# rust-bio/rust-bio

Measured on AMD Instinct MI355X. Metric: GCUPS (SW) + FM-index queries/sec, higher is better.
Workload: dtype int16; 1 GPU; 1000000 x 150 bp synthetic read pairs per GPU, Aligner::local affine-gap (-5,-1,+1,-1), score+coords+traceback ops (BASELINE configs[1]); pairs_per_gpu=1000000, read_len=150, parallelism=shard1

## Files before the change

### rust-bio_amd/csrc/bg_common.h

```cpp
#ifndef BG_COMMON_H
#define BG_COMMON_H
#include <functional>
#include <hip/hip_runtime.h>

#include <cstdint>
#include <cstdlib>
#include <cstdio>
#include <cstring>
#include <string>
#include <vector>

#include "biogpu.h"

extern thread_local std::string bg_tls_error;

#define BG_HIP(call)                                                                     \
    do {                                                                                 \
        hipError_t e__ = (call);                                                         \
        if (e__ != hipSuccess) {                                                         \
            bg_tls_error = std::string(#call) + ": " + hipGetErrorString(e__);           \
            return e__ == hipErrorOutOfMemory ? BG_ERR_OOM : BG_ERR_HIP;                 \
        }                                                                                \
    } while (0)

struct bg_band_scratch;
void bg_band_scratch_free(bg_band_scratch*);
struct bg_seed_scratch;
void bg_seed_scratch_free(bg_seed_scratch*);
struct bg_host_pipe;
void bg_host_pipe_free(bg_host_pipe*);
struct bg_fm_pipe;
void bg_fm_pipe_free(bg_fm_pipe*);
struct bg_myers_scratch;
void bg_myers_scratch_free(bg_myers_scratch*);

struct bg_ctx {
    int device = 0;
    hipStream_t stream = nullptr;
    void* tb = nullptr;
    size_t tb_bytes = 0;
    void* aux = nullptr;
    size_t aux_bytes = 0;
    void* bnd = nullptr;
    size_t bnd_bytes = 0;
    void* io[6] = {};
    size_t io_cap[6] = {};
    void* h_ops = nullptr;
    size_t h_ops_cap = 0;
    void* unpk[2] = {};
    size_t unpk_cap[2] = {};
    void* table = nullptr;
    size_t table_bytes = 0;
    void* sw_table = nullptr;
    size_t sw_table_bytes = 0;
    uint64_t table_hash = 0;
    int table_alpha = 0;
    int32_t* table_matrix = nullptr;
    bg_band_scratch* band = nullptr;
    bg_host_pipe* pipe = nullptr;
    bg_seed_scratch* seed = nullptr;
    bg_fm_pipe* fm_pipe = nullptr;
    bg_myers_scratch* myers = nullptr;
    int64_t myers_chunk_jobs = 0;
    int64_t myers_lds_bytes = 0;
    uint64_t fm_wide_from = 0xFFFFFFFFull;
    uint32_t fm_wide_sb_shift = 17;
    bool fm_host_bytes = false;
    int64_t host_chunk_pairs = 0;
    int64_t chunk_pairs = 0;
    int64_t seed_chunk_reads = 0;
    bool force_wide = false;
    bool no_pk16 = false;
    bool no_local_fast = false;
    bool no_pk16_frame = false;
    bool no_couples = false;
    int band_chain_global = -1;
    bool fq_no_fused = false;
    int sam_lanes = 0;
    int64_t sa_chunk_symbols = 0;
    bool band_chain_rows = true;
    bool band_join_global = false;
    int band_fill_v1 = 0;
    bool band_interior_off = false;
    bool band_packed_off = false;
    int64_t band_packed_thresh = 0;
    int64_t band_budget_gb = 0;
    bool band_on_host = false;
    hipEvent_t scratch_done = nullptr;
    hipStream_t scratch_stream = nullptr;
    bool scratch_used = false;
    bool timing = false;
    hipEvent_t ev[2] = {nullptr, nullptr};
    bg_timing_t last = {};
    uint32_t fill_mask = 0;
    bool fill_framed = false;
};

int bg_reserve(void** p, size_t* cur, size_t need);
int bg_scan_u32(const uint32_t* d_len, uint64_t n, uint64_t* d_off, uint64_t* d_sums, hipStream_t st);
int bg_align_batch_dev_hint(bg_ctx* ctx, const bg_scoring_t* sc, int mode, uint64_t n_pairs, const uint8_t* d_x,
                            const uint64_t* d_x_off, const uint8_t* d_y, const uint64_t* d_y_off, uint32_t max_xlen,
                            uint32_t max_ylen, bg_alignment_t* d_out, uint8_t* d_ops, uint64_t ops_stride, void* stream,
                            int len_hint);

size_t bg_compact_ops_scratch(uint64_t n);
int bg_range_to_host(const uint8_t* d_src, uint8_t* h_dst, const uint64_t* d_slot , hipStream_t st);
int bg_compact_ops_dev(bg_alignment_t* d_rec, uint64_t n, const uint8_t* d_ops, uint8_t* d_compact, bool global_offsets, uint64_t* d_cell,
                       uint64_t* d_batch_total, void* d_scratch, bool long_ops, hipStream_t st);

struct bg_scratch_guard {
    bg_ctx* ctx;
    hipStream_t st;
    bg_scratch_guard(bg_ctx* c, hipStream_t s) : ctx(c), st(s) {
        if (ctx->scratch_used && ctx->scratch_stream != st) hipStreamWaitEvent(st, ctx->scratch_done, 0);
    }
    ~bg_scratch_guard() {
        if (hipEventRecord(ctx->scratch_done, st) == hipSuccess) {
            ctx->scratch_stream = st;
            ctx->scratch_used = true;
        }
    }
};
inline hipError_t bg_copy_pieces(void* dst, const void* src, size_t bytes, hipMemcpyKind kind, hipStream_t st) {
    static const size_t piece = [] {
        const char* e = getenv("BG_COPY_PIECE");
        const long long v = e ? atoll(e) : 0;
        return v > 0 ? (size_t)v : (size_t)(8u << 20);
// ... 29 lines not shown
```

### rust-bio_amd/csrc/core.hip

```cpp
#include <sched.h>

#include <algorithm>
#include <condition_variable>
#include <deque>
#include <mutex>
#include <thread>

#include <cstdlib>

#include "bg_common.h"

thread_local std::string bg_tls_error;

int bg_reserve(void** p, size_t* cur, size_t need) {
    if (need <= *cur) return BG_OK;
    if (*p) {
        hipFree(*p);
        *p = nullptr;
        *cur = 0;
    }
    need = (need + 255) & ~(size_t)255;
    BG_HIP(hipMalloc(p, need));
    *cur = need;
    return BG_OK;
// ... 205 lines not shown
        ctx->band_chain_rows = value != 0;
        return BG_OK;
    }
    if (!strcmp(key, "band_chain_global")) {
        ctx->band_chain_global = (int)value;
        return BG_OK;
    }
    if (!strcmp(key, "band_fill_v1")) {
        ctx->band_fill_v1 = value > 0 ? 1 : value < 0 ? -1 : 0;
        return BG_OK;
    }
    if (!strcmp(key, "band_interior_off")) {
        ctx->band_interior_off = value != 0;
        return BG_OK;
    }
    if (!strcmp(key, "band_packed_off")) {
        ctx->band_packed_off = value != 0;
        return BG_OK;
    }
    if (!strcmp(key, "band_packed_thresh")) {
        if (value < 0 || value > 0xffff) return BG_ERR_INVALID_ARG;
        ctx->band_packed_thresh = value;
        return BG_OK;
    }
    if (!strcmp(key, "band_budget_gb")) {
        if (value < 0 || value > 256) return BG_ERR_INVALID_ARG;
        ctx->band_budget_gb = value;
        return BG_OK;
    }
    if (!strcmp(key, "band_on_host")) {
        ctx->band_on_host = value != 0;
        return BG_OK;
    }
    if (!strcmp(key, "fm_host_bytes")) {
        ctx->fm_host_bytes = value != 0;
        return BG_OK;
    }
    if (!strcmp(key, "host_chunk_pairs")) {
        ctx->host_chunk_pairs = value;
        return BG_OK;
    }
    if (!strcmp(key, "no_couples")) {
        ctx->no_couples = value != 0;
        return BG_OK;
    }
    if (!strcmp(key, "no_local_fast")) {
        ctx->no_local_fast = value != 0;
        return BG_OK;
    }
    if (!strcmp(key, "no_pk16_frame")) {
        ctx->no_pk16_frame = value != 0;
        return BG_OK;
    }
    if (!strcmp(key, "no_pk16")) {
        ctx->no_pk16 = value != 0;
        return BG_OK;
    }
    if (!strcmp(key, "force_wide")) {
        ctx->force_wide = value != 0;
        return BG_OK;
    }
    return BG_ERR_INVALID_ARG;
}

extern "C" int bg_enable_timing(bg_ctx* ctx, int on) {
    if (!ctx) return BG_ERR_INVALID_ARG;
    ctx->timing = on != 0;
    ctx->last = {};
    return BG_OK;
}

extern "C" int bg_last_fill_kernels(bg_ctx* ctx, uint32_t* mask) {
    if (!ctx || !mask) return BG_ERR_INVALID_ARG;
    *mask = ctx->fill_mask;
    return BG_OK;
}

extern "C" int bg_last_fill_framed(bg_ctx* ctx, int* framed) {
    if (!ctx || !framed) return BG_ERR_INVALID_ARG;
    *framed = ctx->fill_framed ? 1 : 0;
    return BG_OK;
}

extern "C" int bg_get_timing(bg_ctx* ctx, bg_timing_t* out) {
    if (!ctx || !out) return BG_ERR_INVALID_ARG;
    *out = ctx->last;
    ctx->last = {};
    return BG_OK;
}

namespace {
__global__ __launch_bounds__(256) void ops_counts_kernel(const bg_alignment_t* __restrict__ rec, uint64_t n, uint32_t* __restrict__ cnt) {
    const uint64_t p = (uint64_t)blockIdx.x * blockDim.x + threadIdx.x;
    if (p < n) cnt[p] = rec[p].status == BG_OK ? rec[p].n_ops : 0u;
}
template <int LANES>
__global__ __launch_bounds__(256) void ops_compact_kernel(bg_alignment_t* __restrict__ rec, uint64_t n, const uint8_t* __restrict__ ops,
                                                          const uint64_t* __restrict__ off, const uint64_t* __restrict__ cell,
                                                          uint8_t* __restrict__ compact, int global_offsets) {
    const uint64_t p = ((uint64_t)blockIdx.x * blockDim.x + threadIdx.x) / LANES;
    const uint32_t l = threadIdx.x % LANES;
    if (p >= n) return;
    const uint32_t k = rec[p].status == BG_OK ? rec[p].n_ops : 0u;
    const uint64_t base = *cell;
    const uint8_t* src = ops + rec[p].ops_off;
    uint8_t* dst = compact + (global_offsets ? base : 0ull) + off[p];
// ... 50 lines not shown
```

### rust-bio_amd/csrc/sw_api.hip

```cpp
#include <algorithm>
#include <chrono>
#include <map>
#include <type_traits>

#include <atomic>
#include <condition_variable>
#include <mutex>
#include <thread>

#include "sw_kernels.h"

namespace bgsw {
void launch_traceback(const SwArgs& a, int nw, hipStream_t st);

static sw_fill_fn sw_fill_get(SwFill f, bool narrow, int lp, int r, int which = 0) {
    static sw_fill_fn (*const get[])(bool, int, int, int) = {
#define BG_X(F) sw_fill_get_##F,
        BG_SW_FILLS(BG_X)
#undef BG_X
    };
    return get[f](narrow, lp, r, which);
}
static int instantiated_r(SwFill f, bool narrow, int lp, int r0, uint32_t m = 0) {
    for (int r = r0; r <= 12; r++)
        if ((!m || m % r == 0) && sw_fill_get(f, narrow, lp, r)) return r;
    return 0;
}

struct Config {
    int lp, r;
};
static Config pick_config(uint32_t m_cap) {
    if (m_cap <= 192) return {16, std::max(2, 2 * (int)((m_cap + 31) / 32))};
    if (m_cap <= 384) return {32, std::max(8, 2 * (int)((m_cap + 63) / 64))};
    return {64, 8};
}

static int64_t score_magnitude(const SwScoring& c, const int32_t* matrix) {
    int64_t mag = std::max<int64_t>(std::abs((int64_t)c.go), std::abs((int64_t)c.ge));
    for (int32_t v : {c.xp, c.xs, c.yp, c.ys})
        if (v != BG_MIN_SCORE) mag = std::max<int64_t>(mag, std::abs((int64_t)v));
    if (matrix) {
        for (size_t t = 0; t < 65536; t++) mag = std::max<int64_t>(mag, std::abs((int64_t)matrix[t]));
    } else {
        mag = std::max<int64_t>(mag, std::max(std::abs((int64_t)c.match), std::abs((int64_t)c.mismatch)));
    }
    return mag;
}

struct FillPlan {
    int lp = 0, r = 0;
    sw_fill_fn fill = nullptr, fill_rest = nullptr, fill_second = nullptr;
    uint32_t tb_fmt = TBF_K1;
    uint32_t fill_bit = 0;
    bool k1p = false, framed = false;
};
static FillPlan plan_fill(const bg_ctx& ctx, const SwScoring& c, int sm, int64_t mag, uint32_t max_xlen, uint32_t max_ylen) {
    const Config cfg = pick_config(max_xlen);
    const bool local = c.xp == 0 && c.xs == 0 && c.yp == 0 && c.ys == 0;
    const bool lf = local && c.go < 0 && c.mismatch < 0 && c.match >= 0 && !ctx.no_local_fast;
    FillPlan p;
    p.lp = cfg.lp;
    if (!ctx.no_pk16 && sm == SCORE_PARAMS && cfg.lp <= 32 && max_xlen >= 1 && mag * ((int64_t)std::max(max_xlen, max_ylen) + 2) <= 2040) {
        const int32_t M = BG_MIN_SCORE;
        SwFill f = lf      ? FILL_K1P_LF
                   : local ? FILL_K1P_LOCAL
// ... 181 lines not shown
using namespace bgsw;

int bg_compact_matrix(const int32_t* matrix, std::vector<uint8_t>& code_map, std::vector<int32_t>& table) {
    return compact_matrix(matrix, code_map, table);
}

static int check_scoring(const bg_scoring_t* sc) {
    if (sc->gap_open > 0 || sc->gap_extend > 0 || sc->xclip_prefix > 0 || sc->xclip_suffix > 0 ||
        sc->yclip_prefix > 0 || sc->yclip_suffix > 0)
        return BG_ERR_POSITIVE_PENALTY;
    return BG_OK;
}

static void reset_fill_report(bg_ctx* ctx) {
    if (!ctx) return;
    ctx->fill_mask = 0;
    ctx->fill_framed = false;
}

static int align_batch_dev_impl(bg_ctx* ctx, const bg_scoring_t* sc, int mode, uint64_t n_pairs,
                                const uint8_t* d_x, const uint64_t* d_x_off, const uint8_t* d_y,
                                const uint64_t* d_y_off, uint32_t max_xlen, uint32_t max_ylen,
                                bg_alignment_t* d_out, uint8_t* d_ops, uint64_t ops_stride,
                                void* stream, int len_hint, const uint8_t* packed_codes = nullptr) {
    if (!ctx || !sc || mode < BG_MODE_CUSTOM || mode > BG_MODE_LOCAL) return BG_ERR_INVALID_ARG;
    int rc = check_scoring(sc);
    if (rc) return rc;
    if (n_pairs == 0) return BG_OK;
    if (!d_x_off || !d_y_off || !d_out) return BG_ERR_INVALID_ARG;
    if (d_ops && ops_stride < (uint64_t)max_xlen + max_ylen + 4) return BG_ERR_OPS_CAP;
    if (max_xlen > (1u << 24) || max_ylen > (1u << 24)) return BG_ERR_TOO_LARGE;
    hipStream_t st = (hipStream_t)stream;
    BG_HIP(hipSetDevice(ctx->device));
    bg_scratch_guard guard(ctx, st);

    SwArgs a = {};
    a.x = d_x;
    a.x_off = d_x_off;
    a.y = d_y;
    a.y_off = d_y_off;
    a.sc = {sc->gap_open,     sc->gap_extend,   sc->xclip_prefix, sc->xclip_suffix,
            sc->yclip_prefix, sc->yclip_suffix, sc->match_score,  sc->mismatch_score};
    if (mode == BG_MODE_GLOBAL) a.sc.xp = a.sc.xs = a.sc.yp = a.sc.ys = BG_MIN_SCORE;
    if (mode == BG_MODE_SEMIGLOBAL) {
        a.sc.xp = a.sc.xs = BG_MIN_SCORE;
        a.sc.yp = a.sc.ys = 0;
    }
    if (mode == BG_MODE_LOCAL) a.sc.xp = a.sc.xs = a.sc.yp = a.sc.ys = 0;
    a.mode = mode;
    a.filter_clips = (mode == BG_MODE_SEMIGLOBAL || mode == BG_MODE_LOCAL);
    a.out = d_out;
    a.ops = d_ops;
    a.ops_stride = ops_stride;

    int sm = SCORE_PARAMS;
    if (sc->matrix) {
        uint64_t h = 0xcbf29ce484222325ull;
        {
            const uint64_t* w = (const uint64_t*)sc->matrix;
            uint64_t h2 = 0x9e3779b97f4a7c15ull;
            for (size_t t = 0; t < 32768; t += 2) {
                h = (h ^ w[t]) * 0x100000001b3ull;
                h2 = (h2 + w[t + 1]) * 0xff51afd7ed558ccdull;
                h2 ^= h2 >> 32;
            }
            h ^= h2;
            if (h == 0) h = 1;
        }
        if (ctx->table_hash != h || !ctx->table_matrix || memcmp(ctx->table_matrix, sc->matrix, 65536 * sizeof(int32_t)) != 0) {
            std::vector<uint8_t> code_map;
            std::vector<int32_t> table;
            const int A = compact_matrix(sc->matrix, code_map, table);
            const size_t bytes = 256 + table.size() * 4;
            ctx->table_hash = 0;
            if (!ctx->table_matrix && !(ctx->table_matrix = (int32_t*)malloc(65536 * sizeof(int32_t)))) return BG_ERR_OOM;
            if ((rc = bg_reserve(&ctx->sw_table, &ctx->sw_table_bytes, bytes))) return rc;
            BG_HIP(hipMemcpyAsync((uint8_t*)ctx->sw_table + 256, table.data(), table.size() * 4,
                                  hipMemcpyHostToDevice, st));
            BG_HIP(hipMemcpyAsync(ctx->sw_table, code_map.data(), 256, hipMemcpyHostToDevice, st));
            BG_HIP(hipStreamSynchronize(st));
            memcpy(ctx->table_matrix, sc->matrix, 65536 * sizeof(int32_t));
            ctx->table_hash = h;
            ctx->table_alpha = A;
        }
        const int A = ctx->table_alpha;
        sm = A <= kMaxLdsAlphabet ? SCORE_LDS : SCORE_GLOBAL;
        a.code_map = (const uint8_t*)ctx->sw_table;
        a.table = (const int32_t*)((uint8_t*)ctx->sw_table + 256);
        a.alpha = A;
    }

    const FillPlan plan = plan_fill(*ctx, a.sc, sm, score_magnitude(a.sc, sc->matrix), max_xlen, max_ylen);
    if (!plan.fill) return BG_ERR_UNSUPPORTED;
    ctx->fill_mask |= plan.fill_bit;
    if (plan.framed) ctx->fill_framed = true;
    if (packed_codes) {
        if (plan.k1p) {
            a.packed = 1;
        } else {
            uint64_t tot[2] = {0, 0};
            BG_HIP(hipMemcpyAsync(&tot[0], d_x_off + n_pairs, 8, hipMemcpyDeviceToHost, st));
            BG_HIP(hipMemcpyAsync(&tot[1], d_y_off + n_pairs, 8, hipMemcpyDeviceToHost, st));
            BG_HIP(hipStreamSynchronize(st));
            for (int k = 0; k < 2; k++)
                if ((rc = bg_reserve(&ctx->unpk[k], &ctx->unpk_cap[k], std::max<uint64_t>(tot[k], 16)))) return rc;
            if ((rc = bg_unpack2_dev(ctx, (const uint32_t*)d_x, tot[0], packed_codes, (uint8_t*)ctx->unpk[0], st))) return rc;
            if ((rc = bg_unpack2_dev(ctx, (const uint32_t*)d_y, tot[1], packed_codes, (uint8_t*)ctx->unpk[1], st))) return rc;
            a.x = (const uint8_t*)ctx->unpk[0];
            a.y = (const uint8_t*)ctx->unpk[1];
        }
    }
    const int nw = tb_words(plan.r);
    const uint32_t pw = 64 / plan.lp;
    SwGeom& g = a.g;
    g.lp = plan.lp;
    g.r = plan.r;
    g.tb_fmt = plan.tb_fmt;
    g.r_inv = (uint32_t)(((1ull << 32) + plan.r - 1) / plan.r);
    g.lp_shift = plan.lp == 16 ? 4 : plan.lp == 32 ? 5 : 6;
    g.m_cap = max_xlen;
    g.n_cap = max_ylen;
    g.nsteps = max_ylen ? max_ylen + plan.lp - 1 : 0;
    g.nstrips = std::max<uint32_t>(1, (max_xlen + plan.lp * plan.r - 1) / (plan.lp * plan.r));
    g.aux_stride = SwGeom::stride_for(max_xlen, max_ylen);

    const size_t tb_per_job = (size_t)tb_job_words(g.nstrips, g.nsteps, nw) * 4;
    const size_t aux_per_pair = (size_t)g.aux_stride * 4;
    const size_t bnd_per_pair = g.nstrips > 1 ? (size_t)(g.n_cap + 1) * 16 : 0;
    const size_t per_pair = tb_per_job / pw + aux_per_pair + bnd_per_pair + 1;
    uint64_t chunk = ctx->chunk_pairs > 0 ? (uint64_t)ctx->chunk_pairs : (1u << 20);
    const uint64_t budget = 48ull << 30;
    chunk = std::min<uint64_t>(chunk, std::max<uint64_t>(pw, budget / per_pair));
    chunk = std::min<uint64_t>(chunk, n_pairs);
    chunk = (chunk + pw - 1) / pw * pw;
    const uint64_t jobs = chunk / pw;
    if ((rc = bg_reserve(&ctx->tb, &ctx->tb_bytes, std::max<size_t>(jobs * tb_per_job, 64)))) return rc;
    if ((rc = bg_reserve(&ctx->aux, &ctx->aux_bytes, chunk * aux_per_pair))) return rc;
    if ((rc = bg_reserve(&ctx->bnd, &ctx->bnd_bytes, std::max<size_t>(chunk * bnd_per_pair, 64)))) return rc;
    a.tb = ctx->tb;
    a.aux = (int32_t*)ctx->aux;
    a.bnd = (int4*)ctx->bnd;
    uint32_t *d_keycnt = nullptr, *d_keysum = nullptr, *d_perm = nullptr, *d_lenst = nullptr;
    if (plan.k1p && !ctx->no_couples) {
        const size_t need = (size_t)kLenKeys * 4 + 1024 * 4 + 64 + chunk * 4;
        if ((rc = bg_reserve(&ctx->bnd, &ctx->bnd_bytes, need))) return rc;
        a.bnd = (int4*)ctx->bnd;
        d_keycnt = (uint32_t*)ctx->bnd;
        d_keysum = d_keycnt + kLenKeys;
        d_lenst = d_keysum + 1024;
        d_perm = d_lenst + 16;
    }

    for (uint64_t p0 = 0; p0 < n_pairs; p0 += chunk) {
        a.pair0 = p0;
        a.n_pairs = (uint32_t)std::min<uint64_t>(chunk, n_pairs - p0);
        const uint32_t njobs = (a.n_pairs + pw - 1) / pw;
        a.perm = nullptr;
        a.len_stats = nullptr;
        a.n_eff = nullptr;
        if (d_perm && a.n_pairs >= 64 && len_hint != 1) {
            const uint32_t* d_st = nullptr;
            if (len_hint < 0) {
                BG_HIP(hipMemsetAsync(d_lenst, 0xff, 8, st));
                BG_HIP(hipMemsetAsync(d_lenst + 2, 0, 8, st));
                sw_len_stats_kernel<<<dim3(std::min<uint32_t>((a.n_pairs + 255) / 256, 256)), dim3(256), 0, st>>>(d_x_off, d_y_off, p0, a.n_pairs, d_lenst);
                d_st = d_lenst;
            }
            BG_HIP(hipMemsetAsync(d_keycnt, 0, (size_t)kLenKeys * 4, st));
            sw_key_hist_kernel<<<dim3((a.n_pairs + 255) / 256), dim3(256), 0, st>>>(d_x_off, d_y_off, p0, a.n_pairs, d_keycnt, d_st);
            sw_key_block_sums_kernel<<<dim3(1024), dim3(256), 0, st>>>(d_keycnt, d_keysum, d_st);
            sw_key_scan_kernel<<<dim3(1024), dim3(1024), 0, st>>>(d_keycnt, d_keysum, d_st);
            sw_key_scatter_kernel<<<dim3((a.n_pairs + 255) / 256), dim3(256), 0, st>>>(d_x_off, d_y_off, p0, a.n_pairs, d_keycnt, d_perm, d_st);
            BG_HIP(hipGetLastError());
            sw_decide_kernel<<<dim3(1), dim3(1), 0, st>>>(d_lenst, a.n_pairs, len_hint < 0 ? -1 : 0, d_lenst + 4);
            a.perm = d_perm;
            a.len_stats = d_st;
            a.n_eff = d_lenst + 4;
        }
        if (ctx->timing) BG_HIP(hipEventRecord(ctx->ev[0], st));
        const uint32_t nwaves = plan.k1p ? (njobs + 1) / 2 : njobs;
        plan.fill<<<dim3((nwaves + 3) / 4), dim3(256), 0, st>>>(a);
        BG_HIP(hipGetLastError());
        if (ctx->timing) BG_HIP(hipEventRecord(ctx->ev[1], st));
        if (plan.fill_rest) plan.fill_rest<<<dim3((nwaves + 3) / 4), dim3(256), 0, st>>>(a);
        if (plan.fill_second && len_hint != 1) plan.fill_second<<<dim3((nwaves + 3) / 4), dim3(256), 0, st>>>(a);
        BG_HIP(hipGetLastError());
        if (ctx->timing) {
            BG_HIP(hipEventSynchronize(ctx->ev[1]));
            float ms = 0;
            BG_HIP(hipEventElapsedTime(&ms, ctx->ev[0], ctx->ev[1]));
            ctx->last.fill_ms += ms;
            ctx->last.fill_launches += 1;
            BG_HIP(hipEventRecord(ctx->ev[0], st));
        }
        launch_traceback(a, nw, st);
        BG_HIP(hipGetLastError());
        if (ctx->timing) {
            BG_HIP(hipEventRecord(ctx->ev[1], st));
            BG_HIP(hipEventSynchronize(ctx->ev[1]));
            float ms = 0;
            BG_HIP(hipEventElapsedTime(&ms, ctx->ev[0], ctx->ev[1]));
            ctx->last.traceback_ms += ms;
            ctx->last.traceback_launches += 1;
        }
    }
    return BG_OK;
}

int bg_align_batch_dev_hint(bg_ctx* ctx, const bg_scoring_t* sc, int mode, uint64_t n_pairs, const uint8_t* d_x,
                            const uint64_t* d_x_off, const uint8_t* d_y, const uint64_t* d_y_off, uint32_t max_xlen,
                            uint32_t max_ylen, bg_alignment_t* d_out, uint8_t* d_ops, uint64_t ops_stride, void* stream,
                            int len_hint) {
    return align_batch_dev_impl(ctx, sc, mode, n_pairs, d_x, d_x_off, d_y, d_y_off, max_xlen, max_ylen, d_out, d_ops, ops_stride,
                                stream, len_hint);
}

extern "C" int bg_align_batch_dev(bg_ctx* ctx, const bg_scoring_t* sc, int mode, uint64_t n_pairs,
                                  const uint8_t* d_x, const uint64_t* d_x_off, const uint8_t* d_y,
                                  const uint64_t* d_y_off, uint32_t max_xlen, uint32_t max_ylen,
                                  bg_alignment_t* d_out, uint8_t* d_ops, uint64_t ops_stride,
                                  void* stream) {
    reset_fill_report(ctx);
    return align_batch_dev_impl(ctx, sc, mode, n_pairs, d_x, d_x_off, d_y, d_y_off, max_xlen, max_ylen, d_out, d_ops, ops_stride, stream, -1);
}

extern "C" int bg_align_batch_packed_dev(bg_ctx* ctx, const bg_scoring_t* sc, int mode, uint64_t n_pairs, const uint32_t* d_x,
                                         const uint64_t* d_x_off, const uint32_t* d_y, const uint64_t* d_y_off,
                                         const uint8_t codes[4], uint32_t max_xlen, uint32_t max_ylen, bg_alignment_t* d_out,
                                         uint8_t* d_ops, uint64_t ops_stride, void* stream) {
    if (!codes || (n_pairs && (!d_x || !d_y))) return BG_ERR_INVALID_ARG;
    for (int a = 0; a < 4; a++)
        for (int b = a + 1; b < 4; b++)
            if (codes[a] == codes[b]) return BG_ERR_INVALID_ARG;
    reset_fill_report(ctx);
    return align_batch_dev_impl(ctx, sc, mode, n_pairs, (const uint8_t*)d_x, d_x_off, (const uint8_t*)d_y, d_y_off, max_xlen, max_ylen,
                                d_out, d_ops, ops_stride, stream, -1, codes);
}

struct bg_host_pipe {
    static constexpr int NSET = 3;
    struct Set {
        uint8_t *h_in = nullptr, *h_out = nullptr;
        uint8_t *d_in = nullptr, *d_out = nullptr;
        uint8_t *d_cmp = nullptr, *d_scan = nullptr;
        size_t in_cap = 0, out_cap = 0, cmp_cap = 0, scan_cap = 0;
        hipEvent_t in_done = nullptr, k_done = nullptr, out_done = nullptr;
    } set[NSET];
    uint64_t* d_cell = nullptr;
// ... 374 lines not shown
```

### rust-bio_amd/csrc/sw_kernels.h

```cpp
#ifndef BG_SW_KERNELS_H
#define BG_SW_KERNELS_H
#include <type_traits>

#include "bg_common.h"

namespace bgsw {

constexpr int32_t NEG = BG_MIN_SCORE;

enum : uint32_t {
    TB_START = 0, TB_INS = 1, TB_DEL = 2, TB_SUBST = 3, TB_MATCH = 4,
    TB_XCLIP_PREFIX = 5, TB_XCLIP_SUFFIX = 6, TB_YCLIP_PREFIX = 7, TB_YCLIP_SUFFIX = 8
};
enum : uint32_t { C_XS = 7, C_MATCH = 6, C_SUBST = 5, C_INS = 3, C_DEL = 2, C_XP = 1, C_YP = 0 };
constexpr int32_t kNarrowFloor = -(1 << 26);
constexpr int32_t kNarrowKeyFloor = (int32_t)0x80000000;

enum { SCORE_PARAMS = 0, SCORE_LDS = 1, SCORE_GLOBAL = 2 };
constexpr int kMaxLdsAlphabet = 64;

struct SwScoring {
    int32_t go, ge, xp, xs, yp, ys;
    int32_t match, mismatch;
};
// ... 24 lines not shown
    uint32_t tb_fmt;
    uint32_t r_inv;
    uint32_t lp_shift;
    __host__ __device__ uint32_t off_Ly() const { return 4; }
    __host__ __device__ uint32_t off_Lx() const { return 4 + (m_cap + 1); }
    __host__ __device__ uint32_t off_bits() const { return 4 + (m_cap + 1) + (n_cap + 1); }
    __host__ __device__ static uint32_t stride_for(uint32_t m_cap, uint32_t n_cap) {
        return 4 + (m_cap + 1) + (n_cap + 1) + (m_cap + 1 + 3) / 4;
    }
};

__device__ __forceinline__ bool len_over(const SwGeom& g, uint32_t m, uint32_t n) { return m > g.m_cap || n > g.n_cap; }

__host__ __device__ constexpr int tb_words(int r) { return (r + 5) / 6; }
__host__ __device__ constexpr uint32_t tb_tile_steps(int nw) { return 16u / (uint32_t)nw; }
__host__ __device__ inline uint64_t tb_job_words(uint32_t nstrips, uint32_t nsteps, int nw) {
    const uint64_t g = (uint64_t)nstrips * nsteps, t = tb_tile_steps(nw);
    return (g + t - 1) / t * 1024ull;
}
__host__ __device__ inline uint64_t tb_word_off(uint64_t g, uint32_t lane, int nw) {
    const uint32_t t = tb_tile_steps(nw);
    return (g / t) * 1024ull + lane * 16u + (uint32_t)(g % t) * (uint32_t)nw;
}

struct SwArgs {
    const uint8_t* x;
    const uint64_t* x_off;
    const uint8_t* y;
    const uint64_t* y_off;
    uint64_t pair0;
    uint32_t n_pairs;
    SwScoring sc;
    const int32_t* table;
    const uint8_t* code_map;
    int32_t alpha;
    void* tb;
    int32_t* aux;
    int4* bnd;
    const uint32_t* perm;
    const uint32_t* len_stats;
    const uint32_t* n_eff;
    __device__ const uint32_t* slot_perm() const {
        if (!perm) return nullptr;
        if (len_stats && len_stats[0] == len_stats[2] && len_stats[1] == len_stats[3]) return nullptr;
        return perm;
    }
    SwGeom g;
    bg_alignment_t* out;
    uint8_t* ops;
    uint64_t ops_stride;
    int32_t mode;
    int32_t filter_clips;
    int32_t packed;
};
__device__ __forceinline__ uint32_t sym2(const uint8_t* stream, uint64_t s) {
    return (((const uint32_t*)stream)[s >> 4] >> (2 * ((uint32_t)s & 15u))) & 3u;
}

struct Col0 {
    int32_t S, I;
    uint32_t sbits, ibits;
};
__device__ __forceinline__ Col0 col0_cell(const SwScoring& sc, uint32_t i, uint32_t m, int32_t fold) {
    Col0 c;
    if (i == 1) {
        c.I = sc.go;
        c.ibits = TB_START;
    } else {
        const int32_t i_score = sc.go + sc.ge * ((int32_t)i - 1);
        const int32_t c_score = sc.xp + sc.go;
        if (i_score > c_score) {
            c.I = i_score;
            c.ibits = TB_INS;
        } else {
            c.I = c_score;
            c.ibits = TB_XCLIP_PREFIX;
        }
    }
    if (i == m) {
        c.S = fold;
        c.sbits = TB_XCLIP_SUFFIX;
    } else {
        c.S = NEG;
        c.sbits = TB_START;
    }
    if (c.I > c.S) {
        c.S = c.I;
        c.sbits = TB_INS;
    }
    if (sc.xp > c.S) {
        c.S = sc.xp;
        c.sbits = TB_XCLIP_PREFIX;
    }
    return c;
}
__device__ __forceinline__ void col0_fold(const SwScoring& sc, uint32_t m, int32_t& fold, uint32_t& lx0) {
    fold = NEG;
    lx0 = 0;
    if (m >= 2) {
        const Col0 c = col0_cell(sc, 1, m, NEG);
        if (c.S + sc.xs > fold) {
            fold = c.S + sc.xs;
            lx0 = m - 1;
        }
    }
}
// ... 71 lines not shown
```

### rust-bio_amd/csrc/sw_traceback.hip

```cpp
#include "sw_kernels.h"

namespace bgsw {

constexpr uint32_t kSegStride = 20;

template <int NW, bool PERM>
__global__ __launch_bounds__(256) __attribute__((amdgpu_waves_per_eu(5, 5))) void sw_traceback_kernel(const SwArgs a) {
    const uint32_t slot = blockIdx.x * blockDim.x + threadIdx.x;
    if (slot >= (a.n_eff ? a.n_eff[PERM ? 1 : 0] : a.n_pairs)) return;
    const uint32_t pair = PERM ? a.perm[slot] : slot;
    const SwScoring sc = a.sc;
    const SwGeom geo = a.g;
    const uint32_t R = geo.r, LP = geo.lp, PW = 64 / geo.lp;

    const uint64_t xo = a.x_off[a.pair0 + pair], yo = a.y_off[a.pair0 + pair];
    const uint32_t m = (uint32_t)(a.x_off[a.pair0 + pair + 1] - xo);
    const uint32_t n = (uint32_t)(a.y_off[a.pair0 + pair + 1] - yo);
    if (len_over(geo, m, n)) {
        bg_alignment_t bad = {};
        bad.xlen = m;
        bad.ylen = n;
        bad.ops_off = (a.pair0 + pair + 1) * a.ops_stride;
        bad.mode = (uint8_t)a.mode;
        bad.status = (int8_t)BG_ERR_INVALID_ARG;
        a.out[a.pair0 + pair] = bad;
        return;
    }

    const int32_t* aux = a.aux + (size_t)slot * geo.aux_stride;
    const int32_t* gLy = aux + geo.off_Ly();
    const int32_t* gLx = aux + geo.off_Lx();
    const uint8_t* bits = (const uint8_t*)(aux + geo.off_bits());
    const uint32_t sbits_m0 = (uint32_t)aux[0];
    const int32_t score = aux[1];
    const uint32_t lxn = (uint32_t)aux[2];

    const uint32_t job = slot / PW, grp = slot % PW;
    const uint32_t* tbj = (const uint32_t*)a.tb + (size_t)job * tb_job_words(geo.nstrips, geo.nsteps, NW);
    __shared__ __align__(16) uint32_t s_seg[256 * kSegStride];
    uint32_t* seg = s_seg + threadIdx.x * kSegStride;
    uint64_t seg_tag = ~0ull;
    auto cell = [&](uint32_t i, uint32_t j) -> uint32_t {
        const uint32_t i1 = i - 1, lrow = __umulhi(i1, geo.r_inv), rr = i1 - lrow * R;
        const uint32_t st = lrow >> geo.lp_shift, llc = lrow & (LP - 1);
        const uint64_t g = (uint64_t)st * geo.nsteps + (j - 1 + llc);
        constexpr uint32_t tsteps = 16 / NW;
        const uint64_t base = (g / tsteps) * 1024ull + (grp * LP + llc) * 16u;
        if (base != seg_tag) {
#pragma unroll
            for (int q = 0; q < 4; q++) *(uint4*)&seg[4 * q] = *(const uint4*)&tbj[base + 4 * q];
            seg_tag = base;
        }
        const uint32_t w = seg[(uint32_t)(g % tsteps) * NW + rr / 6];
        const uint32_t c = rr % 6;
        if (geo.tb_fmt == TBF_K1) return (w >> (5 * c)) & 31u;
        if (geo.tb_fmt == TBF_K1_LF) {
            const uint32_t u = (w >> (5 * c)) & 31u;
            return ((u >> 1) & 7u) | ((~u & 1u) << 3) | (~u & 16u);
        }
        const uint32_t v = (w >> (5 * (c % 3) + 16 * (c / 3))) & 31u;
        const uint32_t mv = (v >> 1) & 7u;
        return ((geo.tb_fmt == TBF_K1P_LF && mv == 0) ? (uint32_t)C_XP : mv) | ((v & 1u) << 3) | (v & 16u);
    };
    auto s_fill = [&](uint32_t i, uint32_t j) -> uint32_t {
        if (j == 0) {
            if (i == 0) return TB_START;
            if (i == m) return sbits_m0;
            return col0_cell(sc, i, m, NEG).sbits;
        }
        if (i == 0) return row0_cell(sc, j).sbits;
        return s_nibble_of_code(cell(i, j) & 7u);
    };
    auto s_nib = [&](uint32_t i, uint32_t j) -> uint32_t {
        if (j == n) return (uint32_t)bits[i] & 15u;
        return s_fill(i, j);
    };
    auto i_nib = [&](uint32_t i, uint32_t j) -> uint32_t {
        if (j == n) return (uint32_t)bits[i] >> 4;
        if (i == 0) return TB_START;
        if (j == 0) return col0_cell(sc, i, m, NEG).ibits;
        return (cell(i, j) & 8u) ? TB_INS : s_fill(i - 1, j);
    };
    auto d_nib = [&](uint32_t i, uint32_t j) -> uint32_t {
        if (j == 0) return TB_START;
        if (i == 0) return row0_cell(sc, j).dbits;
        return (cell(i, j) & 16u) ? TB_DEL : s_fill(i, j - 1);
    };

    uint8_t* ops_end = a.ops ? a.ops + (a.pair0 + pair + 1) * a.ops_stride : nullptr;
    uint32_t n_ops = 0;
    uint32_t clip_len[4] = {0, 0, 0, 0};
    uint32_t n_clips = 0;
    int status = BG_OK;
    const bool dword_ok = ops_end && (((uintptr_t)ops_end & 3) == 0);
    uint32_t acc = 0;
    auto push = [&](uint32_t op) {
        ++n_ops;
        if (!ops_end) return;
        if (dword_ok) {
            acc = (acc << 8) | op;
            if ((n_ops & 3) == 0) *(uint32_t*)(ops_end - n_ops) = acc;
        } else {
            ops_end[-(int64_t)n_ops] = (uint8_t)op;
        }
    };
    auto push_clip = [&](uint32_t op, uint32_t len) {
        if (a.filter_clips) return;
        if (n_clips < 4) clip_len[n_clips] = len;
        else status = BG_ERR_TRACEBACK;
        n_clips++;
        push(op);
    };

    uint32_t i = m, j = n;
    uint32_t xstart = 0, ystart = 0, xend = m, yend = n;
    uint32_t layer = s_nib(m, n);
    const uint32_t guard = 2 * (m + n) + 16;
    uint32_t c_here = 0;
    bool have_c = false;
    for (uint32_t steps = 0; layer != TB_START; steps++) {
        if (steps > guard || (ops_end && n_ops + 1 > a.ops_stride)) {
            status = BG_ERR_TRACEBACK;
            break;
        }
        if (layer >= TB_INS && layer <= TB_MATCH && i >= 1 && i <= m && j >= 1 && j < n) {
            const bool is_ins = layer == TB_INS, is_del = layer == TB_DEL;
            const uint32_t ti = i - (is_del ? 0u : 1u), tj = j - (is_ins ? 0u : 1u);
            if (ti >= 1 && tj >= 1) {
                if (!have_c && (is_ins || is_del)) c_here = cell(i, j);
                const bool ext = (is_ins && (c_here & 8u)) || (is_del && (c_here & 16u));
                push(is_ins ? (uint32_t)BG_OP_INS : is_del ? (uint32_t)BG_OP_DEL : layer == TB_MATCH ? (uint32_t)BG_OP_MATCH : (uint32_t)BG_OP_SUBST);
                c_here = cell(ti, tj);
                have_c = true;
                if (!ext) layer = s_nibble_of_code(c_here & 7u);
                i = ti;
                j = tj;
                continue;
            }
        }
        have_c = false;
        uint32_t next;
        switch (layer) {
            case TB_INS:
                push(BG_OP_INS);
                next = i_nib(i, j);
                i -= 1;
                break;
            case TB_DEL:
                push(BG_OP_DEL);
                next = d_nib(i, j);
                j -= 1;
                break;
            case TB_MATCH:
            case TB_SUBST:
                push(layer == TB_MATCH ? BG_OP_MATCH : BG_OP_SUBST);
                next = (i && j) ? s_nib(i - 1, j - 1) : TB_START;
                i -= 1;
                j -= 1;
                break;
            case TB_XCLIP_PREFIX:
                push_clip(BG_OP_XCLIP, i);
                xstart = i;
                i = 0;
                next = s_nib(0, j);
                break;
            case TB_XCLIP_SUFFIX: {
                if ((geo.tb_fmt == TBF_K1P_LF || geo.tb_fmt == TBF_K1_LF) && j != n) {
                    status = BG_ERR_TRACEBACK;
                    layer = TB_START;
                    continue;
                }
                const uint32_t lx = (j == n) ? lxn
                                    : geo.tb_fmt == TBF_K1 ? (uint32_t)gLx[j]
                                    : geo.lp == 16 ? (uint32_t)((const uint8_t*)gLx)[j] : (uint32_t)((const uint16_t*)gLx)[j];
                push_clip(BG_OP_XCLIP, lx);
                i -= lx;
                xend = i;
                next = i <= m ? s_nib(i, j) : TB_START;
                break;
            }
            case TB_YCLIP_PREFIX:
                push_clip(BG_OP_YCLIP, j);
                ystart = j;
                j = 0;
                next = s_nib(i, 0);
                break;
            default: {
                const uint32_t ly = (uint32_t)gLy[i];
                push_clip(BG_OP_YCLIP, ly);
                j -= ly;
                yend = j;
                next = j <= n ? s_nib(i, j) : TB_START;
                break;
            }
        }
        if (i > m || j > n) {
            status = BG_ERR_TRACEBACK;
            break;
        }
        layer = next;
    }

    if (dword_ok) {
        const uint32_t k = n_ops & 3, done = n_ops - k;
        for (uint32_t t = 0; t < k; t++) ops_end[-(int64_t)(done + t + 1)] = (uint8_t)(acc >> (8 * (k - 1 - t)));
    }
    bg_alignment_t rec;
    rec.score = score;
    rec.xstart = xstart;
    rec.xend = xend;
    rec.ystart = ystart;
    rec.yend = yend;
    rec.xlen = m;
    rec.ylen = n;
    rec.n_ops = n_ops;
    rec.ops_off = (a.pair0 + pair + 1) * a.ops_stride - n_ops;
    const uint32_t nc = n_clips < 4 ? n_clips : 4;
    for (uint32_t c = 0; c < 4; c++) rec.clip_len[c] = c < nc ? clip_len[nc - 1 - c] : 0;
    rec.n_clips = (uint8_t)nc;
    rec.mode = (uint8_t)a.mode;
    rec.status = (int8_t)status;
    rec._pad = 0;
    rec._reserved = 0;
    a.out[a.pair0 + pair] = rec;
}

void launch_traceback(const SwArgs& a, int nw, hipStream_t st) {
    const uint32_t blocks = (a.n_pairs + 255) / 256;
    if (nw == 2)
        sw_traceback_kernel<2, false><<<dim3(blocks), dim3(256), 0, st>>>(a);
    else
        sw_traceback_kernel<1, false><<<dim3(blocks), dim3(256), 0, st>>>(a);
    if (a.perm) {
        if (nw == 2)
            sw_traceback_kernel<2, true><<<dim3(blocks), dim3(256), 0, st>>>(a);
        else
            sw_traceback_kernel<1, true><<<dim3(blocks), dim3(256), 0, st>>>(a);
    }
}

}
```

Baseline: 2188 GCUPS.

## Add fast inner traceback walk with LDS direct loads and format-specialized kernels

Specializes the traceback kernel on the traceback format as a template parameter and adds a tight inner loop for interior match/ins/del moves. The loop tracks row, strip and step indices incrementally instead of recomputing the cell location at each step. Segments are fetched with global_load_lds straight into a wave-shared LDS layout, which frees registers and lets the kernel be capped at 64 VGPRs for higher occupancy. The old path remains available behind a no_tb_walk option. The risks are correctness at strip boundaries and register spills under the VGPR cap.

```diff
diff --git a/rust-bio_amd/csrc/bg_common.h b/rust-bio_amd/csrc/bg_common.h
--- a/rust-bio_amd/csrc/bg_common.h
+++ b/rust-bio_amd/csrc/bg_common.h
@@ -73,6 +73,7 @@
     bool no_pk16 = false;
     bool no_local_fast = false;
     bool no_pk16_frame = false;
+    bool no_tb_walk = false;
     bool no_couples = false;
     int band_chain_global = -1;
     bool fq_no_fused = false;
diff --git a/rust-bio_amd/csrc/core.hip b/rust-bio_amd/csrc/core.hip
--- a/rust-bio_amd/csrc/core.hip
+++ b/rust-bio_amd/csrc/core.hip
@@ -281,6 +281,10 @@
         ctx->no_pk16_frame = value != 0;
         return BG_OK;
     }
+    if (!strcmp(key, "no_tb_walk")) {
+        ctx->no_tb_walk = value != 0;
+        return BG_OK;
+    }
     if (!strcmp(key, "no_pk16")) {
         ctx->no_pk16 = value != 0;
         return BG_OK;
diff --git a/rust-bio_amd/csrc/sw_api.hip b/rust-bio_amd/csrc/sw_api.hip
--- a/rust-bio_amd/csrc/sw_api.hip
+++ b/rust-bio_amd/csrc/sw_api.hip
@@ -11,7 +11,7 @@
 #include "sw_kernels.h"
 
 namespace bgsw {
-void launch_traceback(const SwArgs& a, int nw, hipStream_t st);
+void launch_traceback(const SwArgs& a, int nw, bool walk, hipStream_t st);
 
 static sw_fill_fn sw_fill_get(SwFill f, bool narrow, int lp, int r, int which = 0) {
     static sw_fill_fn (*const get[])(bool, int, int, int) = {
@@ -299,6 +299,7 @@
     a.out = d_out;
     a.ops = d_ops;
     a.ops_stride = ops_stride;
+    a.no_tb_walk = ctx->no_tb_walk;
 
     int sm = SCORE_PARAMS;
     if (sc->matrix) {
@@ -372,6 +373,7 @@
     g.aux_stride = SwGeom::stride_for(max_xlen, max_ylen);
 
     const size_t tb_per_job = (size_t)tb_job_words(g.nstrips, g.nsteps, nw) * 4;
+    if (tb_per_job >= (1ull << 38)) return BG_ERR_TOO_LARGE;
     const size_t aux_per_pair = (size_t)g.aux_stride * 4;
     const size_t bnd_per_pair = g.nstrips > 1 ? (size_t)(g.n_cap + 1) * 16 : 0;
     const size_t per_pair = tb_per_job / pw + aux_per_pair + bnd_per_pair + 1;
@@ -440,7 +442,7 @@
             ctx->last.fill_launches += 1;
             BG_HIP(hipEventRecord(ctx->ev[0], st));
         }
-        launch_traceback(a, nw, st);
+        launch_traceback(a, nw, !a.no_tb_walk, st);
         BG_HIP(hipGetLastError());
         if (ctx->timing) {
             BG_HIP(hipEventRecord(ctx->ev[1], st));
diff --git a/rust-bio_amd/csrc/sw_kernels.h b/rust-bio_amd/csrc/sw_kernels.h
--- a/rust-bio_amd/csrc/sw_kernels.h
+++ b/rust-bio_amd/csrc/sw_kernels.h
@@ -100,6 +100,7 @@
     int32_t mode;
     int32_t filter_clips;
     int32_t packed;
+    int32_t no_tb_walk;
 };
 __device__ __forceinline__ uint32_t sym2(const uint8_t* stream, uint64_t s) {
     return (((const uint32_t*)stream)[s >> 4] >> (2 * ((uint32_t)s & 15u))) & 3u;
diff --git a/rust-bio_amd/csrc/sw_traceback.hip b/rust-bio_amd/csrc/sw_traceback.hip
--- a/rust-bio_amd/csrc/sw_traceback.hip
+++ b/rust-bio_amd/csrc/sw_traceback.hip
@@ -4,8 +4,28 @@
 
 constexpr uint32_t kSegStride = 20;
 
-template <int NW, bool PERM>
-__global__ __launch_bounds__(256) __attribute__((amdgpu_waves_per_eu(5, 5))) void sw_traceback_kernel(const SwArgs a) {
+constexpr uint64_t cell_shifts(uint32_t fmt) {
+    uint64_t v = 0;
+    for (uint32_t rr = 0; rr < 12; rr++) {
+        const uint32_t c = rr % 6;
+        const uint64_t sh = (fmt == TBF_K1 || fmt == TBF_K1_LF) ? 5 * c : 5 * (c % 3) + 16 * (c / 3);
+        v |= sh << (5 * rr);
+    }
+    return v;
+}
+constexpr uint32_t move_nibbles(uint32_t fmt) {
+    uint32_t v = 0;
+    for (uint32_t k = 0; k < 8; k++) {
+        const uint32_t code = (fmt == TBF_K1P_LF && k == 0) ? (uint32_t)C_XP : k;
+        const uint32_t nib = code == C_MATCH ? TB_MATCH : code == C_SUBST ? TB_SUBST : code == C_INS ? TB_INS : code == C_DEL ? TB_DEL
+                             : code == C_XP ? TB_XCLIP_PREFIX : code == C_YP ? TB_YCLIP_PREFIX : TB_XCLIP_SUFFIX;
+        v |= nib << (4 * k);
+    }
+    return v;
+}
+
+template <int NW, bool PERM, uint32_t FMT, bool WALK>
+__device__ __forceinline__ void sw_traceback_body(const SwArgs& a) {
     const uint32_t slot = blockIdx.x * blockDim.x + threadIdx.x;
     if (slot >= (a.n_eff ? a.n_eff[PERM ? 1 : 0] : a.n_pairs)) return;
     const uint32_t pair = PERM ? a.perm[slot] : slot;
@@ -31,41 +51,52 @@
     const int32_t* gLy = aux + geo.off_Ly();
     const int32_t* gLx = aux + geo.off_Lx();
     const uint8_t* bits = (const uint8_t*)(aux + geo.off_bits());
-    const uint32_t sbits_m0 = (uint32_t)aux[0];
-    const int32_t score = aux[1];
-    const uint32_t lxn = (uint32_t)aux[2];
 
     const uint32_t job = slot / PW, grp = slot % PW;
     const uint32_t* tbj = (const uint32_t*)a.tb + (size_t)job * tb_job_words(geo.nstrips, geo.nsteps, NW);
-    __shared__ __align__(16) uint32_t s_seg[256 * kSegStride];
-    uint32_t* seg = s_seg + threadIdx.x * kSegStride;
-    uint64_t seg_tag = ~0ull;
+    __shared__ __align__(16) uint32_t s_seg[WALK ? 256 * 16 : 256 * kSegStride];
+    uint32_t* seg = WALK ? s_seg + (threadIdx.x & ~63u) * 16 + (threadIdx.x & 63u) * 4 : s_seg + threadIdx.x * kSegStride;
+    uint32_t seg_tag = ~0u;
+    const uint32_t lane0 = grp * LP;
+    auto fetch = [&](uint32_t tag) {
+        const uint32_t* src = tbj + (uint64_t)tag * 16u;
+        if constexpr (WALK) {
+            uint32_t* wave_seg = s_seg + (threadIdx.x & ~63u) * 16;
+#pragma unroll
+            for (int q = 0; q < 4; q++)
+                __builtin_amdgcn_global_load_lds((const __attribute__((address_space(1))) void*)(src + 4 * q),
+                                                 (__attribute__((address_space(3))) void*)(wave_seg + 256 * q), 16, 0, 0);
+            __builtin_amdgcn_s_waitcnt(0x0F70);
+            asm volatile("" ::: "memory");
+        } else {
+#pragma unroll
+            for (int q = 0; q < 4; q++) *(uint4*)&seg[4 * q] = *(const uint4*)&src[4 * q];
+        }
+        seg_tag = tag;
+    };
     auto cell = [&](uint32_t i, uint32_t j) -> uint32_t {
         const uint32_t i1 = i - 1, lrow = __umulhi(i1, geo.r_inv), rr = i1 - lrow * R;
         const uint32_t st = lrow >> geo.lp_shift, llc = lrow & (LP - 1);
         const uint64_t g = (uint64_t)st * geo.nsteps + (j - 1 + llc);
         constexpr uint32_t tsteps = 16 / NW;
-        const uint64_t base = (g / tsteps) * 1024ull + (grp * LP + llc) * 16u;
-        if (base != seg_tag) {
-#pragma unroll
-            for (int q = 0; q < 4; q++) *(uint4*)&seg[4 * q] = *(const uint4*)&tbj[base + 4 * q];
-            seg_tag = base;
-        }
-        const uint32_t w = seg[(uint32_t)(g % tsteps) * NW + rr / 6];
+        const uint32_t tag = (uint32_t)(g / tsteps) * 64u + (lane0 + llc);
+        if (tag != seg_tag) fetch(tag);
+        const uint32_t k = (uint32_t)(g % tsteps) * NW + rr / 6;
+        const uint32_t w = WALK ? seg[(k >> 2) * 256 + (k & 3u)] : seg[k];
         const uint32_t c = rr % 6;
-        if (geo.tb_fmt == TBF_K1) return (w >> (5 * c)) & 31u;
-        if (geo.tb_fmt == TBF_K1_LF) {
+        if (FMT == TBF_K1) return (w >> (5 * c)) & 31u;
+        if (FMT == TBF_K1_LF) {
             const uint32_t u = (w >> (5 * c)) & 31u;
             return ((u >> 1) & 7u) | ((~u & 1u) << 3) | (~u & 16u);
         }
         const uint32_t v = (w >> (5 * (c % 3) + 16 * (c / 3))) & 31u;
         const uint32_t mv = (v >> 1) & 7u;
-        return ((geo.tb_fmt == TBF_K1P_LF && mv == 0) ? (uint32_t)C_XP : mv) | ((v & 1u) << 3) | (v & 16u);
+        return ((FMT == TBF_K1P_LF && mv == 0) ? (uint32_t)C_XP : mv) | ((v & 1u) << 3) | (v & 16u);
     };
     auto s_fill = [&](uint32_t i, uint32_t j) -> uint32_t {
         if (j == 0) {
             if (i == 0) return TB_START;
-            if (i == m) return sbits_m0;
+            if (i == m) return (uint32_t)aux[0];
             return col0_cell(sc, i, m, NEG).sbits;
         }
         if (i == 0) return row0_cell(sc, j).sbits;
@@ -119,11 +150,52 @@
     uint32_t c_here = 0;
     bool have_c = false;
     for (uint32_t steps = 0; layer != TB_START; steps++) {
+        if constexpr (WALK) {
+            if (layer - TB_INS <= TB_MATCH - TB_INS && j < n && i > (layer != TB_DEL ? 1u : 0u) && j > (layer != TB_INS ? 1u : 0u) &&
+                (!ops_end || (uint64_t)n_ops + i + j <= a.ops_stride)) {
+                constexpr uint32_t tsteps = 16 / NW, ts_shift = NW == 2 ? 3 : 4;
+                uint32_t rr, llc, g;
+                auto locate = [&]() {
+                    const uint32_t i1 = i - 1, lrow = __umulhi(i1, geo.r_inv);
+                    rr = i1 - lrow * R;
+                    llc = lrow & (LP - 1);
+                    g = (lrow >> geo.lp_shift) * geo.nsteps + (j - 1 + llc);
+                };
+                auto raw = [&]() -> uint32_t {
+                    const uint32_t tag = (g >> ts_shift) * 64u + (lane0 + llc);
+                    if (tag != seg_tag) fetch(tag);
+                    const uint32_t k = (g & (tsteps - 1)) * NW + (NW == 2 && rr >= 6 ? 1u : 0u);
+                    const uint32_t w = seg[(k >> 2) * 256 + (k & 3u)];
+                    return (w >> ((uint32_t)(cell_shifts(FMT) >> (5 * rr)) & 31u)) & 31u;
+                };
+                constexpr bool move_first = FMT == TBF_K1;
+                constexpr uint32_t ibit = move_first ? 8u : 1u;
+                constexpr uint32_t ext_set = FMT == TBF_K1_LF ? 0u : ~0u;
+                locate();
+                uint32_t e = 1;
+                for (;;) {
+                    const uint32_t c = raw();
+                    if (!e) layer = (move_nibbles(FMT) >> (move_first ? (c & 7u) << 2 : (c << 1) & 28u)) & 15u;
+                    const uint32_t di = layer != TB_DEL ? 1u : 0u, dj = layer != TB_INS ? 1u : 0u;
+                    if (!((layer - TB_INS <= TB_MATCH - TB_INS) & (i > di) & (j > dj))) break;
+                    e = (c ^ ~ext_set) & (dj ? (di ? 0u : 16u) : ibit);
+                    push(TB_MATCH - layer);
+                    const uint32_t wrap = di & (rr == 0 ? 1u : 0u);
+                    const bool strip = FMT == TBF_K1 && (wrap & (llc == 0 ? 1u : 0u));
+                    i -= di;
+                    j -= dj;
+                    rr = wrap ? R - 1 : rr - di;
+                    llc -= wrap;
+                    g -= dj + wrap;
+                    if (strip) locate();
+                }
+            }
+        }
         if (steps > guard || (ops_end && n_ops + 1 > a.ops_stride)) {
             status = BG_ERR_TRACEBACK;
             break;
         }
-        if (layer >= TB_INS && layer <= TB_MATCH && i >= 1 && i <= m && j >= 1 && j < n) {
+        if (!WALK && layer >= TB_INS && layer <= TB_MATCH && i >= 1 && i <= m && j >= 1 && j < n) {
             const bool is_ins = layer == TB_INS, is_del = layer == TB_DEL;
             const uint32_t ti = i - (is_del ? 0u : 1u), tj = j - (is_ins ? 0u : 1u);
             if (ti >= 1 && tj >= 1) {
@@ -165,13 +237,13 @@
                 next = s_nib(0, j);
                 break;
             case TB_XCLIP_SUFFIX: {
-                if ((geo.tb_fmt == TBF_K1P_LF || geo.tb_fmt == TBF_K1_LF) && j != n) {
+                if ((FMT == TBF_K1P_LF || FMT == TBF_K1_LF) && j != n) {
                     status = BG_ERR_TRACEBACK;
                     layer = TB_START;
                     continue;
                 }
-                const uint32_t lx = (j == n) ? lxn
-                                    : geo.tb_fmt == TBF_K1 ? (uint32_t)gLx[j]
+                const uint32_t lx = (j == n) ? (uint32_t)aux[2]
+                                    : FMT == TBF_K1 ? (uint32_t)gLx[j]
                                     : geo.lp == 16 ? (uint32_t)((const uint8_t*)gLx)[j] : (uint32_t)((const uint16_t*)gLx)[j];
                 push_clip(BG_OP_XCLIP, lx);
                 i -= lx;
@@ -206,7 +278,7 @@
         for (uint32_t t = 0; t < k; t++) ops_end[-(int64_t)(done + t + 1)] = (uint8_t)(acc >> (8 * (k - 1 - t)));
     }
     bg_alignment_t rec;
-    rec.score = score;
+    rec.score = aux[1];
     rec.xstart = xstart;
     rec.xend = xend;
     rec.ystart = ystart;
@@ -225,18 +297,40 @@
     a.out[a.pair0 + pair] = rec;
 }
 
-void launch_traceback(const SwArgs& a, int nw, hipStream_t st) {
+template <int NW, bool PERM, uint32_t FMT>
+__global__ __launch_bounds__(256) __attribute__((amdgpu_waves_per_eu(5, 8), amdgpu_num_vgpr(64))) void sw_traceback_kernel(const SwArgs a) {
+    sw_traceback_body<NW, PERM, FMT, true>(a);
+}
+template <int NW, bool PERM, uint32_t FMT>
+__global__ __launch_bounds__(256) __attribute__((amdgpu_waves_per_eu(5, 5))) void sw_traceback_kernel_nowalk(const SwArgs a) {
+    sw_traceback_body<NW, PERM, FMT, false>(a);
+}
+
+template <int NW, uint32_t FMT, bool WALK>
+static void launch_k2(const SwArgs& a, hipStream_t st) {
     const uint32_t blocks = (a.n_pairs + 255) / 256;
-    if (nw == 2)
-        sw_traceback_kernel<2, false><<<dim3(blocks), dim3(256), 0, st>>>(a);
+    if constexpr (WALK) {
+        sw_traceback_kernel<NW, false, FMT><<<dim3(blocks), dim3(256), 0, st>>>(a);
+        if (a.perm) sw_traceback_kernel<NW, true, FMT><<<dim3(blocks), dim3(256), 0, st>>>(a);
+    } else {
+        sw_traceback_kernel_nowalk<NW, false, FMT><<<dim3(blocks), dim3(256), 0, st>>>(a);
+        if (a.perm) sw_traceback_kernel_nowalk<NW, true, FMT><<<dim3(blocks), dim3(256), 0, st>>>(a);
+    }
+}
+template <int NW, bool WALK>
+static void launch_k2_fmt(const SwArgs& a, hipStream_t st) {
+    switch (a.g.tb_fmt) {
+        case TBF_K1: return launch_k2<NW, TBF_K1, WALK>(a, st);
+        case TBF_K1_LF: return launch_k2<NW, TBF_K1_LF, WALK>(a, st);
+        case TBF_K1P: return launch_k2<NW, TBF_K1P, WALK>(a, st);
+        default: return launch_k2<NW, TBF_K1P_LF, WALK>(a, st);
+    }
+}
+void launch_traceback(const SwArgs& a, int nw, bool walk, hipStream_t st) {
+    if (walk)
+        nw == 2 ? launch_k2_fmt<2, true>(a, st) : launch_k2_fmt<1, true>(a, st);
     else
-        sw_traceback_kernel<1, false><<<dim3(blocks), dim3(256), 0, st>>>(a);
-    if (a.perm) {
-        if (nw == 2)
-            sw_traceback_kernel<2, true><<<dim3(blocks), dim3(256), 0, st>>>(a);
-        else
-            sw_traceback_kernel<1, true><<<dim3(blocks), dim3(256), 0, st>>>(a);
-    }
-}
-
-}
+        nw == 2 ? launch_k2_fmt<2, false>(a, st) : launch_k2_fmt<1, false>(a, st);
+}
+
+}
```

Result: no change. 2169 GCUPS (-0.9%).
